# tensorlayer/TLXCV

Measured on AMD Instinct MI355X. Metric: images/sec fwd, higher is better.
Workload: dtype f16; 1 GPU; ResNet-50 fp16 forward, 224x224, batch 256 per GPU (BASELINE configs[1]); global_batch=256, per_gpu_batch=256, weights=seeded random (tlxcv_amd.seeded, seed 1), parallelism=single GPU, launch=hipGraph replay of the forward

## Files before the change

include/tlxmi.h:

```cpp
#ifndef TLXMI_H
#define TLXMI_H

#include <stddef.h>
#include <stdint.h>

#ifdef __cplusplus
extern "C" {
#endif

#define TLXMI_VERSION 101

typedef enum tlxmi_status {
    TLXMI_OK = 0,
    TLXMI_ERR_BAD_ARG = -1,
    TLXMI_ERR_UNSUPPORTED = -2,
    TLXMI_ERR_ALIGNMENT = -3,
    TLXMI_ERR_LAUNCH = -4,
    TLXMI_ERR_NO_DEVICE = -5
} tlxmi_status;

typedef enum tlxmi_dtype { TLXMI_F16 = 0, TLXMI_F32 = 1 } tlxmi_dtype;

typedef enum tlxmi_act {
    TLXMI_ACT_NONE = 0,
// ... 72 lines not shown
    int32_t N, H, W, C;
    int32_t out_h, out_w;
    int32_t kh, kw;
    int32_t out_dtype;
    int32_t layout;
    int32_t fold_b, cpad;
    int32_t normalize;
} tlxmi_preproc_desc;
size_t tlxmi_preprocess_u8_workspace_bytes(const tlxmi_preproc_desc* d);
int tlxmi_preprocess_u8(const tlxmi_preproc_desc* d, const void* images, const int32_t* xbounds, const int32_t* xk,
                        const int32_t* ybounds, const int32_t* yk, const float* mean, const float* std_, void* workspace,
                        void* out, void* stream);

int tlxmi_preprocess_linear_u8(const tlxmi_preproc_desc* d, const void* images, const int32_t* xidx, const int32_t* xcoef,
                               const int32_t* yidx, const int32_t* ycoef, const float* mean, const float* std_, void* out,
                               void* stream);

typedef struct tlxmi_seam_desc {
    int32_t dtype;
    int64_t rows;
    int32_t K1, N1, N2;
    int32_t t2_ld, skip_ld, y_ld, t1_ld;
    int32_t act;
} tlxmi_seam_desc;
int tlxmi_bottleneck_seam_supported(int dtype, int K1, int N1, int N2);
int tlxmi_bottleneck_seam_proj(const tlxmi_seam_desc* d, const void* t2, const void* w3_packed, const float* scale3,
                               const float* shift3, const void* x, const void* wd_packed, const float* scale_d,
                               const float* shift_d, void* y, const void* w1_packed, const float* scale1,
                               const float* shift1, void* t1, void* stream);
int tlxmi_bottleneck_seam(const tlxmi_seam_desc* d, const void* t2, const void* w3_packed, const float* scale3,
                          const float* shift3, const void* skip, void* y, const void* w1_packed, const float* scale1,
                          const float* shift1, void* t1, void* stream);
int tlxmi_bottleneck_seam_dec_supported(int dtype, int K1, int N1, int N2, int64_t rows, int H, int W);
int tlxmi_bottleneck_seam_dec(const tlxmi_seam_desc* d, int H, int W, const void* t2, const void* w3_packed, const float* scale3,
                              const float* shift3, const void* skip, void* y, const void* w1_packed, const float* scale1,
                              const float* shift1, void* t1, void* stream);

typedef struct tlxmi_proj_desc {
    int32_t dtype;
    int32_t N, Ho, Wo;
    int32_t K1, K2, Cout;
    int32_t H2, W2, stride;
    int32_t x_ld, x2_ld, y_ld;
    int32_t act;
    float act_param;
    uint32_t flags;
} tlxmi_proj_desc;
int tlxmi_conv1x1_proj_supported(const tlxmi_proj_desc* d, const void* x, const void* x2, const void* w_packed, const void* y);
// ... 266 lines not shown
```

tlxcv_amd/_lib.py:

```python
import ctypes as C
import os

_HERE = os.path.dirname(os.path.abspath(__file__))
LIB_PATH = os.path.join(_HERE, "libtlxmi.so")

F16, F32 = 0, 1
ACT_NONE, ACT_RELU, ACT_RELU6, ACT_LEAKY, ACT_HARDSWISH, ACT_HARDSIGMOID, ACT_GELU, ACT_SIGMOID, ACT_SILU = range(9)
EPI_RES_AFTER_ACT = 1
EPI_MAXPOOL_3S2P1 = 4
PLAN_SHARED_HALF = 0x100
PLAN_SHARED_FULL = 0x200
LAYOUT_NHWC, LAYOUT_NCHW = 0, 1


class ConvDesc(C.Structure):
    _fields_ = [(n, C.c_int32) for n in (
        "dtype", "N", "H", "W", "C", "Cout", "R", "S", "stride_h", "stride_w", "pad_h", "pad_w",
        "dil_h", "dil_w", "Ho", "Wo", "x_ld", "y_ld", "res_ld", "y_nstride", "res_nstride", "act")] + [
        ("act_param", C.c_float), ("flags", C.c_uint32)]


class DwConvDesc(C.Structure):
    _fields_ = [(n, C.c_int32) for n in (
        "dtype", "N", "H", "W", "C", "R", "S", "stride_h", "stride_w", "pad_h", "pad_w", "dil_h",
# ... 50 lines not shown
            "q_batch_stride", "q_row_stride", "k_batch_stride", "k_row_stride", "v_batch_stride", "v_row_stride",
            "out_batch_stride", "out_row_stride")]


class LevitAttnDesc(C.Structure):
    _fields_ = [(n, C.c_int32) for n in ("dtype", "B", "heads", "kd", "d", "Rq", "Rk", "stride")] + [("scale", C.c_float), ("act", C.c_int32)] + [
        (n, C.c_int64) for n in ("q_batch_stride", "q_row_stride", "q_head_stride", "k_batch_stride", "k_row_stride", "k_head_stride",
                                 "v_batch_stride", "v_row_stride", "v_head_stride", "out_batch_stride", "out_row_stride")]


class TntInnerDesc(C.Structure):
    _fields_ = [(n, C.c_int32) for n in ("dtype", "patches", "pixels", "dim", "heads", "hidden")] + [
        (n, C.c_float) for n in ("scale", "eps1", "eps2", "eps3")] + [(n, C.c_int64) for n in ("x_row_stride", "y_row_stride", "yn_row_stride")]


class GsaBlockDesc(C.Structure):
    _fields_ = [(n, C.c_int32) for n in ("dtype", "B", "Lq", "Lk", "C", "heads")] + [(n, C.c_float) for n in ("scale", "eps")] + [
        (n, C.c_int64) for n in ("x_batch_stride", "x_row_stride", "k_batch_stride", "k_row_stride", "v_batch_stride", "v_row_stride",
                                 "y_batch_stride", "y_row_stride")]


class SeamDesc(C.Structure):
    _fields_ = [("dtype", C.c_int32), ("rows", C.c_int64)] + [(n, C.c_int32) for n in (
        "K1", "N1", "N2", "t2_ld", "skip_ld", "y_ld", "t1_ld", "act")]


class ProjDesc(C.Structure):
    _fields_ = [(n, C.c_int32) for n in ("dtype", "N", "Ho", "Wo", "K1", "K2", "Cout", "H2", "W2", "stride", "x_ld", "x2_ld", "y_ld", "act")] + [
        ("act_param", C.c_float), ("flags", C.c_uint32)]


class PreprocDesc(C.Structure):
    _fields_ = [(n, C.c_int32) for n in ("N", "H", "W", "C", "out_h", "out_w", "kh", "kw", "out_dtype", "layout", "fold_b",
                                         "cpad", "normalize")]


_vp, _i, _f, _u, _l = C.c_void_p, C.c_int, C.c_float, C.c_uint32, C.c_int64

PROTOTYPES = {
    "tlxmi_nchw_to_nhwc": [_vp, _i, _vp, _i, _i, _i, _i, _i, _i, _vp],
    "tlxmi_nchw_to_nhwc_s2d": [_vp, _i, _vp, _i, _i, _i, _i, _i, _i, _i, _vp],
    "tlxmi_patchify": [_vp, _i, _vp, _i, _i, _i, _i, _i, _i, _i, _vp],
    "tlxmi_patch_embed4": [_vp, _i, _vp, _vp, _vp, _vp, _vp, _i, _i, _i, _i, _f, _vp],
    "tlxmi_patch_embed4_pos": [_vp, _i, _vp, _vp, _vp, _vp, _vp, _vp, _i, _i, _i, _i, _f, _vp],
    "tlxmi_nhwc_to_nchw": [_vp, _i, _i, _vp, _i, _i, _i, _i, _i, _vp],
    "tlxmi_pack_filter": [_vp, _vp, _i, _i, _i, _i, _i, _vp],
    "tlxmi_fold_bn": [_vp, _vp, _vp, _vp, _vp, _f, _i, _vp, _vp, _vp],
# ... 53 lines not shown
    "tlxmi_preact_conv1x1": [_i, _l, _i, _i, _i, _i, _vp, _vp, _vp, _i, _vp, _vp, _vp, _i, _vp, _vp],
    "tlxmi_lka_dw": [C.POINTER(LkaDwDesc), _vp, _vp, _vp, _vp, _vp, _vp, _vp],
    "tlxmi_lka_gate": [C.POINTER(LkaGateDesc), _vp, _vp, _vp, _vp, _vp, _vp, _vp, _vp, _vp, _vp, _vp, _vp],
    "tlxmi_mul": [_vp, _vp, _vp, _i, _l, _i, _i, _i, _i, _vp],
    "tlxmi_shuffle_unit": [C.POINTER(ShuffleUnitDesc), _vp, _vp, _vp, _vp],
    "tlxmi_shuffle_concat": [_vp, _vp, _vp, _i, _l, _i, _i, _i, _i, _vp],
    "tlxmi_ghost_module": [C.POINTER(GhostModuleDesc), _vp, _vp, _vp, _vp, _vp],
    "tlxmi_mixconv_dw": [C.POINTER(MixConvDwDesc), _vp, _vp, _vp, _vp, _vp],
}
_SPECIAL = {
    "tlxmi_version": ([], C.c_int),
    "tlxmi_last_error": ([], C.c_char_p),
    "tlxmi_device_count": ([], C.c_int),
    "tlxmi_packed_filter_bytes": ([_i, _i, _i, _i, _i], C.c_size_t),
    "tlxmi_packed_group_filter_bytes": ([_i, _i, _i, _i, _i, _i], C.c_size_t),
    "tlxmi_group_conv_chunks": ([_i, _i, _i, _i], C.c_int),
    "tlxmi_group_conv2d_small_supported": ([C.POINTER(ConvDesc), _i], C.c_int),
    "tlxmi_conv2d_maxpool_supported": ([C.POINTER(ConvDesc)], C.c_int),
    "tlxmi_conv2d_splitk_supported": ([C.POINTER(ConvDesc), _i], C.c_int),
    "tlxmi_preprocess_u8_workspace_bytes": ([C.POINTER(PreprocDesc)], C.c_size_t),
    "tlxmi_multiclass_nms_workspace_bytes": ([_i, _i], C.c_size_t),
    "tlxmi_bottleneck_seam_supported": ([_i, _i, _i, _i], C.c_int),
    "tlxmi_bottleneck_seam_dec_supported": ([_i, _i, _i, _i, _l, _i, _i], C.c_int),
    "tlxmi_conv1x1_proj_supported": ([C.POINTER(ProjDesc), _vp, _vp, _vp, _vp], C.c_int),
    "tlxmi_linear_ln_supported": ([_i, _l, _i, _i, _i, _i], C.c_int),
    "tlxmi_mlp_seam_supported": ([_i, _i, _i, _i], C.c_int),
    "tlxmi_sepconv2d_supported": ([C.POINTER(SepConvDesc)], C.c_int),
    "tlxmi_dwconv7_stats_supported": ([C.POINTER(DwConv7Desc)], C.c_int),
    "tlxmi_preact_conv1x1_supported": ([_i, _l, _i, _i, _i, _i, _i, _i], C.c_int),
    "tlxmi_sr_attention_supported": ([C.POINTER(MhaDesc)], C.c_int),
    "tlxmi_cswin_attention_supported": ([C.POINTER(CswinAttnDesc)], C.c_int),
    "tlxmi_levit_attention_supported": ([C.POINTER(LevitAttnDesc)], C.c_int),
    "tlxmi_tnt_inner_supported": ([C.POINTER(TntInnerDesc)], C.c_int),
    "tlxmi_tnt_inner_param_count": ([_i, _i], C.c_size_t),
    "tlxmi_gsa_block_supported": ([C.POINTER(GsaBlockDesc)], C.c_int),
    "tlxmi_gsa_block_param_count": ([_i], C.c_size_t),
    "tlxmi_lka_dw_supported": ([C.POINTER(LkaDwDesc)], C.c_int),
    "tlxmi_lka_gate_supported": ([C.POINTER(LkaGateDesc)], C.c_int),
    "tlxmi_shuffle_unit_supported": ([C.POINTER(ShuffleUnitDesc)], C.c_int),
    "tlxmi_shuffle_unit_param_bytes": ([_i], C.c_size_t),
    "tlxmi_ghost_module_supported": ([C.POINTER(GhostModuleDesc)], C.c_int),
    "tlxmi_ghost_module_param_bytes": ([_i, _i], C.c_size_t),
    "tlxmi_mixconv_dw_supported": ([C.POINTER(MixConvDwDesc), _i], C.c_int),
    "tlxmi_mixconv_dw_param_bytes": ([C.POINTER(MixConvDwDesc)], C.c_size_t),
}
ALL_SYMBOLS = sorted(list(PROTOTYPES) + list(_SPECIAL))
# ... 71 lines not shown
```

tlxcv_amd/csrc/block_seam.h:

```cpp
#pragma once
#include <hip/hip_runtime.h>

namespace tlxmi {

struct SeamArgs {
    const char *x, *w3, *res, *w1;
    char *y, *z;
    const float *scale3, *shift3, *scale1, *shift1;
    int M, N1;
    int x_ld, res_ld, y_ld, z_ld;
    unsigned x_bytes, w3_bytes, res_bytes, y_bytes, w1_bytes, z_bytes;
    int y_nt, z_nt;
    const char* wd;
    const float *scale_d, *shift_d;
    unsigned wd_bytes;
    int debug;
};

struct SeamDecArgs : SeamArgs {
    int HW, W;
};

bool block_seam_shape_ok(int K1, int N1, int N2);
int launch_block_seam(const SeamArgs& a, int K1, int N2, hipStream_t st);
int launch_block_seam_dec(const SeamDecArgs& a, int K1, int N2, hipStream_t st);
int launch_mlp_seam(const SeamArgs& a, int K1, int N2, hipStream_t st);

}
```

tlxcv_amd/csrc/block_seam.hip:

```cpp
#include "kernel_util.h"
#include <stdio.h>
#include "block_seam.h"
#include <type_traits>
#ifdef TLXMI_TUNING
#define TLXMI_DBG_NT(x) (x)
#else
#define TLXMI_DBG_NT(x) (false)
#endif

namespace tlxmi {

static __device__ __forceinline__ int bs_f1(int r) { return ((r >> 1) & 1) | (((r >> 4) & 3) << 1); }
static __device__ __forceinline__ int bs_f2(int r) { return (((r >> 1) & 1) << 2) | ((r >> 5) & 1); }

static __device__ __forceinline__ unsigned bs_pkrelu(unsigned v) {
    unsigned r;
    asm("v_pk_max_f16 %0, %1, 0" : "=v"(r) : "v"(v));
    return r;
}
static __device__ __forceinline__ u32x2 bs_bn_skip_relu4(f32x4 acc, f32x4 sc, f32x4 sh, half4v skip) {
    f32x2 t0 = f32x2{__builtin_fmaf(acc[0], sc[0], (float)skip[0]), __builtin_fmaf(acc[1], sc[1], (float)skip[1])};
    f32x2 t1 = f32x2{__builtin_fmaf(acc[2], sc[2], (float)skip[2]), __builtin_fmaf(acc[3], sc[3], (float)skip[3])};
    t0 += f32x2{sh[0], sh[1]};
    t1 += f32x2{sh[2], sh[3]};
// ... 263 lines not shown
        for (int h = 0; h < 2; ++h) {
            const f32x4 s0 = *reinterpret_cast<const f32x4*>(sc + 8 * h), s1 = *reinterpret_cast<const f32x4*>(sc + 8 * h + 4);
            const f32x4 h0 = *reinterpret_cast<const f32x4*>(sh + 8 * h), h1 = *reinterpret_cast<const f32x4*>(sh + 8 * h + 4);
#pragma unroll
            for (int pw = 0; pw < PW; ++pw) {
                u32x2 o0, o1;
                if constexpr (MLP) {
                    const half8v rv = __builtin_bit_cast(half8v, buf_load16(rsrd, pok[pw] ? (pix[pw] * a.res_ld + 64 * q + 16 * g + 8 * h) * 2 : BUF_OOB));
                    o0 = bs_bn_res4(acc2[4 * q + 2 * h][pw], s0, h0, half4v{rv[0], rv[1], rv[2], rv[3]});
                    o1 = bs_bn_res4(acc2[4 * q + 2 * h + 1][pw], s1, h1, half4v{rv[4], rv[5], rv[6], rv[7]});
                } else {
                    o0 = bs_bn_relu4(acc2[4 * q + 2 * h][pw], s0, h0);
                    o1 = bs_bn_relu4(acc2[4 * q + 2 * h + 1][pw], s1, h1);
                }
                const u32x4 o = u32x4{o0[0], o0[1], o1[0], o1[1]};
                if (TLXMI_DBG(a, 4)) continue;
                if (TLXMI_DBG_NT(a.z_nt)) buf_store16<BUF_NT>(zsrd, o, pok[pw] ? (pix[pw] * a.z_ld + 64 * q + 16 * g + 8 * h) * 2 : BUF_OOB);
                else buf_store16(zsrd, o, pok[pw] ? (pix[pw] * a.z_ld + 64 * q + 16 * g + 8 * h) * 2 : BUF_OOB);
            }
        }
    }
}

template <int K1, int N2, int NW>
__global__ __launch_bounds__(64 * NW, 1) void seam_pair_kernel(const SeamArgs a) {
    static_assert(N2 % 128 == 0 && NW % 2 == 0, "pairs of waves split N2 in halves of whole 64-channel blocks");
    constexpr int NT = 64 * NW;
    constexpr int IPT = 512 / NT;
    constexpr int PW = 2;
    constexpr int KS = K1 / 32;
    constexpr int CB = K1 / 64;
    constexpr int Q2 = N2 / 64;
    constexpr int NP = CB + Q2;
    constexpr int T2H = N2 / 32;
    constexpr int PANEL = 64 * 128;
    extern __shared__ __attribute__((aligned(16))) char smem[];
    char* const wbuf = smem;
    float* const tab3 = reinterpret_cast<float*>(smem + 2 * NP * PANEL);
    float* const tab1 = tab3 + 2 * a.N1;
    char* const ybuf = reinterpret_cast<char*>(tab1 + 2 * N2);

    const int t = threadIdx.x, lane = t & 63;
    const int wid = __builtin_amdgcn_readfirstlane(t >> 6);
    const int hh = wid & 1, pp = wid >> 1;
    const int fr = lane & 15, g = lane >> 4;

// ... 414 lines not shown
static int launch_seam_t(const std::conditional_t<DEC, SeamDecArgs, SeamArgs>& a, hipStream_t st) {
    constexpr int NP = K1 / 64 + N2 / 64 + (PROJ ? K1 / 64 : 0);
    const size_t lds = (size_t)2 * NP * 64 * 128 + (size_t)(2 * a.N1 + 2 * N2 + (PROJ ? 2 * a.N1 : 0)) * sizeof(float);
    if (lds > 160 * 1024) return fail(TLXMI_ERR_UNSUPPORTED, "block_seam: %zu bytes of LDS", lds);
    const void* fn = reinterpret_cast<const void*>(&seam_kernel<K1, N2, PW, NW, PROJ, WPS, MLP, DEC>);
    if (lds > 64 * 1024)
        if (int rc = raise_lds_limit(fn, 160 * 1024, "block_seam")) return rc;
    const long grid = ((long)a.M + NW * 16 * PW - 1) / (NW * 16 * PW);
    if (grid >= (1l << 31)) return fail(TLXMI_ERR_UNSUPPORTED, "block_seam: too many rows");
#ifdef TLXMI_TUNING
    if (tune_int("TLXMI_SEAM_OCC", 0)) {
        int nb = -1;
        hipError_t oe = hipOccupancyMaxActiveBlocksPerMultiprocessor(&nb, fn, 64 * NW, lds);
        fprintf(stderr, "seam<%d,%d,%d,%d,%d>: lds %zu, grid %ld, occupancy %d workgroups / CU (%s)\n", K1, N2, PW, NW, (int)PROJ, lds, grid, nb, hipGetErrorString(oe));
    }
#endif
    auto b = a;
    void* args[] = {&b};
    hipError_t e = hipLaunchKernel(fn, dim3((unsigned)grid), dim3(64 * NW), args, lds, st);
    if (e != hipSuccess) return fail(TLXMI_ERR_LAUNCH, "block_seam: HIP launch failed: %s", hipGetErrorString(e));
    return TLXMI_OK;
}

bool block_seam_shape_ok(int K1, int N1, int N2) {
    if (N1 % 64 || N1 < 64 || N1 > 2048) return false;
    if (!((K1 == 64 && (N2 == 64 || N2 == 128)) || (K1 == 128 && (N2 == 128 || N2 == 256)) || (K1 == 256 && N2 == 256))) return false;
    const size_t lds = (size_t)2 * (K1 / 64 + N2 / 64) * 64 * 128 + (size_t)(2 * N1 + 2 * N2) * sizeof(float) + (K1 == 256 ? (size_t)8 * 2 * 1024 : 0);
    return lds <= 160 * 1024;
}

int launch_mlp_seam(const SeamArgs& a0, int K1, int N2, hipStream_t st) {
    SeamArgs b = a0;
    b.z_nt = b.y_nt = 0;
    b.debug = 0;
    if (K1 == 128 && N2 == 128) return launch_seam_t<128, 128, 2, 8, false, 0, true>(b, st);
    return fail(TLXMI_ERR_UNSUPPORTED, "mlp_seam: no instantiation for %d -> N1 -> %d channels", K1, N2);
}

int launch_block_seam(const SeamArgs& a0, int K1, int N2, hipStream_t st) {
    const int vv = (int)tune_int("TLXMI_SEAM", 0);
    const int v = vv & 1;
    SeamArgs b = a0;
    b.z_nt = (vv & 2) ? 1 : 0;
    b.y_nt = (vv & 4) ? 1 : 0;
    b.debug = (int)tune_int("TLXMI_SEAM_DBG", 0);
    const SeamArgs& a = b;
    if (a.wd) {
        if (K1 == 64 && N2 == 64) return launch_seam_t<64, 64, 2, 4, true>(a, st);
        return fail(TLXMI_ERR_UNSUPPORTED, "block_seam: the projection-shortcut form is compiled for 64 -> N1 -> 64 channels");
    }
    if (vv & 16) {
        if (K1 == 64 && N2 == 64) return launch_seam_t<64, 64, 2, 4, false, 3>(a, st);
        if (K1 == 64 && N2 == 128) return launch_seam_t<64, 128, 2, 4, false, 3>(a, st);
        if (K1 == 128 && N2 == 128) return launch_seam_t<128, 128, 2, 4, false, 2>(a, st);
    }
    if (K1 == 64 && N2 == 64) return v ? launch_seam_t<64, 64, 2, 8>(a, st) : launch_seam_t<64, 64, 2, 4>(a, st);
    if (K1 == 64 && N2 == 128) return v ? launch_seam_t<64, 128, 2, 8>(a, st) : launch_seam_t<64, 128, 2, 4>(a, st);
    if (K1 == 128 && N2 == 128) return v ? launch_seam_t<128, 128, 2, 4>(a, st) : launch_seam_t<128, 128, 2, 8>(a, st);
    if (K1 == 128 && N2 == 256) return v ? launch_seam_t<128, 256, 1, 4>(a, st) : launch_seam_t<128, 256, 1, 8>(a, st);
    if (K1 == 256 && N2 == 256) {
#ifdef TLXMI_TUNING
        if (vv & 64) return launch_seam_pair_t<256, 256, 8, !SEAM_PAIR_ANTIPHASE>(a, st);
#endif
        if (!(vv & 32)) return launch_seam_pair_t<256, 256, 8, SEAM_PAIR_ANTIPHASE>(a, st);
        return v ? launch_seam_t<256, 256, 1, 4>(a, st) : launch_seam_t<256, 256, 1, 8>(a, st);
    }
    return fail(TLXMI_ERR_UNSUPPORTED, "block_seam: no instantiation for %d -> N1 -> %d channels", K1, N2);
}

static bool block_seam_dec_shape_ok(int K1, int N1, int N2) {
    return ((K1 == 64 && N1 == 256 && N2 == 128) || (K1 == 128 && N1 == 512 && N2 == 256)) && block_seam_shape_ok(K1, N1, N2);
}

int launch_block_seam_dec(const SeamDecArgs& a0, int K1, int N2, hipStream_t st) {
    SeamDecArgs b = a0;
    b.z_nt = b.y_nt = 0;
    b.debug = 0;
    if (K1 == 64 && N2 == 128) return launch_seam_t<64, 128, 2, 4, false, 0, false, true>(b, st);
    if (K1 == 128 && N2 == 256) return launch_seam_t<128, 256, 1, 8, false, 0, false, true>(b, st);
    return fail(TLXMI_ERR_UNSUPPORTED, "block_seam_dec: no instantiation for %d -> N1 -> %d channels", K1, N2);
}

}

using namespace tlxmi;

extern "C" int tlxmi_bottleneck_seam_supported(int dtype, int K1, int N1, int N2) {
    return dtype == TLXMI_F16 && block_seam_shape_ok(K1, N1, N2) ? 1 : 0;
}

static int seam_impl(const tlxmi_seam_desc* d, const void* t2, const void* w3_packed, const float* scale3,
                     const float* shift3, const void* skip, void* y, const void* w1_packed, const float* scale1,
                     const float* shift1, void* t1, void* stream, const void* wd_packed, const float* scale_d, const float* shift_d) {
    TLXMI_REQUIRE(d && t2 && w3_packed && skip && y && w1_packed && t1, TLXMI_ERR_BAD_ARG, "bottleneck_seam: null argument");
    TLXMI_REQUIRE(d->dtype == TLXMI_F16, TLXMI_ERR_UNSUPPORTED, "bottleneck_seam: fp16 only (the fp32 parity mode runs the two convolutions)");
    TLXMI_REQUIRE(d->rows > 0 && d->K1 > 0 && d->N1 > 0 && d->N2 > 0, TLXMI_ERR_BAD_ARG, "bottleneck_seam: bad extent");
    if (!block_seam_shape_ok(d->K1, d->N1, d->N2))
        return fail(TLXMI_ERR_UNSUPPORTED, "bottleneck_seam: no kernel for %d -> %d -> %d channels", d->K1, d->N1, d->N2);
    TLXMI_REQUIRE(d->t2_ld >= d->K1 && d->skip_ld >= (wd_packed ? d->K1 : d->N1) && d->y_ld >= d->N1 && d->t1_ld >= d->N2, TLXMI_ERR_BAD_ARG, "bottleneck_seam: row stride below the channel count");
    TLXMI_REQUIRE(!wd_packed || (aligned16(wd_packed) && d->K1 == 64 && d->N2 == 64), TLXMI_ERR_UNSUPPORTED, "bottleneck_seam_proj: 64 -> N1 -> 64 channels only");
    TLXMI_REQUIRE(d->t2_ld % 8 == 0 && d->skip_ld % 8 == 0 && d->y_ld % 8 == 0 && d->t1_ld % 8 == 0 && aligned16(t2) && aligned16(skip) && aligned16(y) &&
                      aligned16(t1) && aligned16(w3_packed) && aligned16(w1_packed),
                  TLXMI_ERR_ALIGNMENT, "bottleneck_seam: rows must be whole 16-byte chunks");
    TLXMI_REQUIRE(d->act == TLXMI_ACT_RELU, TLXMI_ERR_UNSUPPORTED, "bottleneck_seam: ReLU after both convolutions only");
    const long long rows = d->rows;
    const long long big = (1ll << 31);
    TLXMI_REQUIRE(rows * d->t2_ld * 2 < big && rows * d->skip_ld * 2 < big && rows * d->y_ld * 2 < big && rows * d->t1_ld * 2 < big && rows < big,
                  TLXMI_ERR_UNSUPPORTED, "bottleneck_seam: a tensor exceeds the 2 GiB the 32-bit buffer offsets address");
    SeamArgs a;
    a.x = (const char*)t2; a.w3 = (const char*)w3_packed; a.res = (const char*)skip; a.w1 = (const char*)w1_packed;
    a.y = (char*)y; a.z = (char*)t1;
    a.scale3 = scale3; a.shift3 = shift3; a.scale1 = scale1; a.shift1 = shift1;
    a.M = (int)rows; a.N1 = d->N1;
    a.x_ld = d->t2_ld; a.res_ld = d->skip_ld; a.y_ld = d->y_ld; a.z_ld = d->t1_ld;
    a.x_bytes = (unsigned)(rows * d->t2_ld * 2); a.res_bytes = (unsigned)(rows * d->skip_ld * 2);
    a.y_bytes = (unsigned)(rows * d->y_ld * 2); a.z_bytes = (unsigned)(rows * d->t1_ld * 2);
    a.wd = (const char*)wd_packed; a.scale_d = scale_d; a.shift_d = shift_d;
    a.wd_bytes = wd_packed ? (unsigned)(((size_t)(d->N1 + 127) / 128 * 128) * (size_t)d->K1 * 2) : 0u;
    a.w3_bytes = (unsigned)(((size_t)(d->N1 + 127) / 128 * 128) * (size_t)d->K1 * 2);
    a.w1_bytes = (unsigned)(((size_t)(d->N2 + 127) / 128 * 128) * (size_t)d->N1 * 2);
    const int rc = launch_block_seam(a, d->K1, d->N2, as_stream(stream));
    if (rc != TLXMI_OK) return rc;
    return check_launch("bottleneck_seam");
}

extern "C" int tlxmi_bottleneck_seam(const tlxmi_seam_desc* d, const void* t2, const void* w3_packed, const float* scale3,
                                     const float* shift3, const void* skip, void* y, const void* w1_packed, const float* scale1,
                                     const float* shift1, void* t1, void* stream) {
    return seam_impl(d, t2, w3_packed, scale3, shift3, skip, y, w1_packed, scale1, shift1, t1, stream, nullptr, nullptr, nullptr);
}

extern "C" int tlxmi_bottleneck_seam_proj(const tlxmi_seam_desc* d, const void* t2, const void* w3_packed, const float* scale3,
                                          const float* shift3, const void* x, const void* wd_packed, const float* scale_d,
                                          const float* shift_d, void* y, const void* w1_packed, const float* scale1,
                                          const float* shift1, void* t1, void* stream) {
    TLXMI_REQUIRE(wd_packed, TLXMI_ERR_BAD_ARG, "bottleneck_seam_proj: null shortcut filter");
    return seam_impl(d, t2, w3_packed, scale3, shift3, x, y, w1_packed, scale1, shift1, t1, stream, wd_packed, scale_d, shift_d);
}

static long long seam_dec_rows(long long rows, int H, int W) { return rows / ((long long)H * W) * ((H + 1) / 2) * ((W + 1) / 2); }

extern "C" int tlxmi_bottleneck_seam_dec_supported(int dtype, int K1, int N1, int N2, int64_t rows, int H, int W) {
    if (dtype != TLXMI_F16 || !block_seam_dec_shape_ok(K1, N1, N2) || rows <= 0 || H <= 0 || W <= 0) return 0;
    const long long big = (1ll << 31), hw = (long long)H * W;
// ... 12 lines not shown
    const long long big = (1ll << 31), rows = d->rows, hw = (long long)H * W;
    TLXMI_REQUIRE(hw < big && rows % hw == 0, TLXMI_ERR_BAD_ARG, "bottleneck_seam_dec: rows is not a whole number of H x W images");
    TLXMI_REQUIRE(d->t2_ld >= d->K1 && d->skip_ld >= d->N1 && d->y_ld >= d->N1 && d->t1_ld >= d->N2, TLXMI_ERR_BAD_ARG, "bottleneck_seam_dec: row stride below the channel count");
    TLXMI_REQUIRE(d->t2_ld % 8 == 0 && d->skip_ld % 8 == 0 && d->y_ld % 8 == 0 && d->t1_ld % 8 == 0 && aligned16(t2) && aligned16(skip) && aligned16(y) &&
                      aligned16(t1) && aligned16(w3_packed) && aligned16(w1_packed),
                  TLXMI_ERR_ALIGNMENT, "bottleneck_seam_dec: rows must be whole 16-byte chunks");
    TLXMI_REQUIRE(d->act == TLXMI_ACT_RELU, TLXMI_ERR_UNSUPPORTED, "bottleneck_seam_dec: ReLU after both convolutions only");
    const long long yrows = seam_dec_rows(rows, H, W);
    TLXMI_REQUIRE(rows * d->t2_ld * 2 < big && rows * d->skip_ld * 2 < big && yrows * d->y_ld * 2 < big && rows * d->t1_ld * 2 < big,
                  TLXMI_ERR_UNSUPPORTED, "bottleneck_seam_dec: a tensor exceeds the 2 GiB the 32-bit buffer offsets address");
    SeamDecArgs a;
    a.x = (const char*)t2; a.w3 = (const char*)w3_packed; a.res = (const char*)skip; a.w1 = (const char*)w1_packed;
    a.y = (char*)y; a.z = (char*)t1;
    a.scale3 = scale3; a.shift3 = shift3; a.scale1 = scale1; a.shift1 = shift1;
    a.M = (int)rows; a.N1 = d->N1;
    a.x_ld = d->t2_ld; a.res_ld = d->skip_ld; a.y_ld = d->y_ld; a.z_ld = d->t1_ld;
    a.x_bytes = (unsigned)(rows * d->t2_ld * 2); a.res_bytes = (unsigned)(rows * d->skip_ld * 2);
    a.y_bytes = (unsigned)(yrows * d->y_ld * 2); a.z_bytes = (unsigned)(rows * d->t1_ld * 2);
    a.wd = nullptr; a.scale_d = a.shift_d = nullptr; a.wd_bytes = 0;
    a.w3_bytes = (unsigned)(((size_t)(d->N1 + 127) / 128 * 128) * (size_t)d->K1 * 2);
    a.w1_bytes = (unsigned)(((size_t)(d->N2 + 127) / 128 * 128) * (size_t)d->N1 * 2);
    a.y_nt = a.z_nt = 0; a.debug = 0;
    a.HW = (int)hw; a.W = W;
    const int rc = launch_block_seam_dec(a, d->K1, d->N2, as_stream(stream));
    if (rc != TLXMI_OK) return rc;
    return check_launch("bottleneck_seam_dec");
}

extern "C" int tlxmi_mlp_seam_supported(int dtype, int K, int hidden, int N) {
    return (dtype == TLXMI_F16 && K == 128 && N == 128 && hidden % 64 == 0 && hidden >= 64 && hidden <= 2048 && block_seam_shape_ok(K, hidden, N)) ? 1 : 0;
}

extern "C" int tlxmi_mlp_seam(int dtype, int64_t rows, int K, int hidden, int N, const void* x, int x_ld, const void* w1_packed, const float* bias1,
                              const void* w2_packed, const float* bias2, const void* res, int res_ld, void* out, int out_ld, void* stream) {
    TLXMI_REQUIRE(x && w1_packed && w2_packed && res && out, TLXMI_ERR_BAD_ARG, "mlp_seam: null argument");
    if (!tlxmi_mlp_seam_supported(dtype, K, hidden, N)) return fail(TLXMI_ERR_UNSUPPORTED, "mlp_seam: no kernel for %d -> %d -> %d", K, hidden, N);
    TLXMI_REQUIRE(rows > 0 && x_ld >= K && res_ld >= N && out_ld >= N, TLXMI_ERR_BAD_ARG, "mlp_seam: bad extent");
    TLXMI_REQUIRE(x_ld % 8 == 0 && res_ld % 8 == 0 && out_ld % 8 == 0 && aligned16(x) && aligned16(res) && aligned16(out) && aligned16(w1_packed) && aligned16(w2_packed),
                  TLXMI_ERR_ALIGNMENT, "mlp_seam: rows must be whole 16-byte chunks");
    const long long big = (1ll << 31);
    TLXMI_REQUIRE(rows * x_ld * 2 < big && rows * res_ld * 2 < big && rows * out_ld * 2 < big, TLXMI_ERR_UNSUPPORTED, "mlp_seam: a tensor exceeds 2 GiB");
    SeamArgs a;
    a.x = (const char*)x; a.w3 = (const char*)w1_packed; a.res = (const char*)res; a.w1 = (const char*)w2_packed;
    a.y = nullptr; a.z = (char*)out;
    a.scale3 = nullptr; a.shift3 = bias1; a.scale1 = nullptr; a.shift1 = bias2;
    a.M = (int)rows; a.N1 = hidden;
    a.x_ld = x_ld; a.res_ld = res_ld; a.y_ld = 0; a.z_ld = out_ld;
// ... 10 lines not shown
```

tlxcv_amd/engine.py:

```python
import ctypes as C
import threading

import torch

from . import _lib
from ._lib import (ACT_GELU, ACT_HARDSIGMOID, ACT_HARDSWISH, ACT_LEAKY, ACT_NONE, ACT_RELU, ACT_RELU6,
                   ACT_SIGMOID, ACT_SILU, EPI_RES_AFTER_ACT, F16, F32)

EPI_RES_BCAST_N = 2

_precision = torch.float16

_options = {"splitk": True,
            "attn_comb": True,
            "seams": True,
            "seam256": True,
            "proj_fold": 7,
            "seam_decimate": True,
            "two_streams": True,
            "conv_splitk": True,
            "patch_linear": True,
            "patch_embed4": True,
            "mlp_seam": True,
            "lnfold": True,
# ... 554 lines not shown


def bottleneck_seam_supported(K1, N1, N2, dtype):
    return bool(_lib.load().tlxmi_bottleneck_seam_supported(dt_code(dtype), int(K1), int(N1), int(N2)))


def bottleneck_seam_dec_supported(K1, N1, N2, rows, H, W, dtype):
    return bool(_lib.load().tlxmi_bottleneck_seam_dec_supported(dt_code(dtype), int(K1), int(N1), int(N2), int(rows), int(H), int(W)))


def bottleneck_seam(t2, pk3, scale3, shift3, skip, pk1, scale1, shift1, proj=None, y_stride2=False):
    need_gpu(t2, "input")
    N, H, W, ld = t2.shape
    if y_stride2 and proj is not None:
        raise RuntimeError("bottleneck_seam: no decimated form of the projection-shortcut seam")
    if skip.shape[:3] != t2.shape[:3] or skip.dtype != t2.dtype or not skip.is_contiguous() or not t2.is_contiguous():
        raise RuntimeError("bottleneck_seam: t2 / skip must be dense NHWC maps of one dtype and extent")
    y = torch.empty((N, (H + 1) // 2, (W + 1) // 2, pk3.Cout) if y_stride2 else (N, H, W, pk3.Cout), dtype=t2.dtype, device=t2.device)
    t1 = torch.empty((N, H, W, pk1.Cout), dtype=t2.dtype, device=t2.device)
    rows = N * H * W
    if getattr(_tls, "act_max", None) is not None:
        _note_act(t2.numel() * t2.element_size(), skip.numel() * skip.element_size(), y.numel() * y.element_size(), t1.numel() * t1.element_size())
    d = _lib.SeamDesc(dtype=dt_code(t2.dtype), rows=rows, K1=pk3.Cin, N1=pk3.Cout, N2=pk1.Cout, t2_ld=ld, skip_ld=skip.shape[-1],
                      y_ld=pk3.Cout, t1_ld=pk1.Cout, act=ACT_RELU)
    if y_stride2:
        name = "tlxmi_bottleneck_seam_dec"
        args = (C.byref(d), H, W, _p(t2), _p(pk3.buf), _p(scale3), _p(shift3), _p(skip), _p(y), _p(pk1.buf), _p(scale1), _p(shift1), _p(t1), _stream())
    elif proj is None:
        name = "tlxmi_bottleneck_seam"
        args = (C.byref(d), _p(t2), _p(pk3.buf), _p(scale3), _p(shift3), _p(skip), _p(y), _p(pk1.buf), _p(scale1), _p(shift1), _p(t1), _stream())
    else:
        name = "tlxmi_bottleneck_seam_proj"
        pkd, sd, hd = proj
        args = (C.byref(d), _p(t2), _p(pk3.buf), _p(scale3), _p(shift3), _p(skip), _p(pkd.buf), _p(sd), _p(hd), _p(y), _p(pk1.buf), _p(scale1),
                _p(shift1), _p(t1), _stream())
    if _probe is None:
        _lib.call(name, *args)
        return y, t1
    es = t2.element_size()
    skip_ch = pk3.Cout if proj is None else proj[0].Cin
    alg_bytes = (rows * (pk3.Cin + skip_ch + pk1.Cout) + y.numel() + pk3.Cout * pk3.Cin + pk1.Cout * pk1.Cin) * es
    flops = 2 * rows * (pk3.Cout * pk3.Cin + pk1.Cout * pk1.Cin + (0 if proj is None else pk3.Cout * proj[0].Cin))
    e0, e1 = torch.cuda.Event(enable_timing=True), torch.cuda.Event(enable_timing=True)
    e0.record()
    _lib.call(name, *args)
    e1.record()
    _probe.append((e0, e1, alg_bytes, flops, (N, H, W, pk3.Cin, pk3.Cout, pk1.Cout, "seam+dec" if y_stride2 else "seam" if proj is None else "seam+proj", True)))
# ... 1745 lines not shown
```

Measured before the change: 80760 images/sec.

## Add persistent LDS-resident-weight bottleneck seam kernel for K1=64 stages

Adds a persistent kernel for the bottleneck seam (1x1 conv3 + BN + skip + ReLU fused with the next block's 1x1 conv1). It stages all filter panels and BN tables into up to 160 KiB of LDS once per workgroup, then grid-strides over 32-row tiles with prefetched activations and skip data. The aim is to stop reloading weights per tile and to cut launch/occupancy overhead for the K1=64 plain, projection and decimated forms. It is selected by default unless a shared-plan flag is set. The cost is one resident workgroup per CU and a large LDS footprint, which may limit latency hiding.

```diff
diff --git a/include/tlxmi.h b/include/tlxmi.h
--- a/include/tlxmi.h
+++ b/include/tlxmi.h
@@ -118,8 +118,10 @@
     int32_t K1, N1, N2;
     int32_t t2_ld, skip_ld, y_ld, t1_ld;
     int32_t act;
+    uint32_t flags;
 } tlxmi_seam_desc;
 int tlxmi_bottleneck_seam_supported(int dtype, int K1, int N1, int N2);
+int tlxmi_bottleneck_seam_resident(int dtype, int K1, int N1, int N2, int form);
 int tlxmi_bottleneck_seam_proj(const tlxmi_seam_desc* d, const void* t2, const void* w3_packed, const float* scale3,
                                const float* shift3, const void* x, const void* wd_packed, const float* scale_d,
                                const float* shift_d, void* y, const void* w1_packed, const float* scale1,
diff --git a/tlxcv_amd/_lib.py b/tlxcv_amd/_lib.py
--- a/tlxcv_amd/_lib.py
+++ b/tlxcv_amd/_lib.py
@@ -96,7 +96,7 @@
 
 class SeamDesc(C.Structure):
     _fields_ = [("dtype", C.c_int32), ("rows", C.c_int64)] + [(n, C.c_int32) for n in (
-        "K1", "N1", "N2", "t2_ld", "skip_ld", "y_ld", "t1_ld", "act")]
+        "K1", "N1", "N2", "t2_ld", "skip_ld", "y_ld", "t1_ld", "act")] + [("flags", C.c_uint32)]
 
 
 class ProjDesc(C.Structure):
@@ -196,6 +196,7 @@
     "tlxmi_multiclass_nms_workspace_bytes": ([_i, _i], C.c_size_t),
     "tlxmi_bottleneck_seam_supported": ([_i, _i, _i, _i], C.c_int),
     "tlxmi_bottleneck_seam_dec_supported": ([_i, _i, _i, _i, _l, _i, _i], C.c_int),
+    "tlxmi_bottleneck_seam_resident": ([_i, _i, _i, _i, _i], C.c_int),
     "tlxmi_conv1x1_proj_supported": ([C.POINTER(ProjDesc), _vp, _vp, _vp, _vp], C.c_int),
     "tlxmi_linear_ln_supported": ([_i, _l, _i, _i, _i, _i], C.c_int),
     "tlxmi_mlp_seam_supported": ([_i, _i, _i, _i], C.c_int),
diff --git a/tlxcv_amd/csrc/block_seam.h b/tlxcv_amd/csrc/block_seam.h
--- a/tlxcv_amd/csrc/block_seam.h
+++ b/tlxcv_amd/csrc/block_seam.h
@@ -22,8 +22,8 @@
 };
 
 bool block_seam_shape_ok(int K1, int N1, int N2);
-int launch_block_seam(const SeamArgs& a, int K1, int N2, hipStream_t st);
-int launch_block_seam_dec(const SeamDecArgs& a, int K1, int N2, hipStream_t st);
+int launch_block_seam(const SeamArgs& a, int K1, int N2, bool shared, hipStream_t st);
+int launch_block_seam_dec(const SeamDecArgs& a, int K1, int N2, bool shared, hipStream_t st);
 int launch_mlp_seam(const SeamArgs& a, int K1, int N2, hipStream_t st);
 
 }
diff --git a/tlxcv_amd/csrc/block_seam.hip b/tlxcv_amd/csrc/block_seam.hip
--- a/tlxcv_amd/csrc/block_seam.hip
+++ b/tlxcv_amd/csrc/block_seam.hip
@@ -309,6 +309,264 @@
     }
 }
 
+template <int N2, int NW, bool PROJ, bool DEC>
+__global__ __launch_bounds__(64 * NW, 1) void seam_res_kernel(const std::conditional_t<DEC, SeamDecArgs, SeamArgs> a) {
+    static_assert(!(PROJ && DEC), "one form at a time");
+    static_assert(NW >= 8, "the first 512 threads stage the filters");
+    constexpr int K1 = 64;
+    constexpr int PW = 2;
+    constexpr int NT = 64 * NW;
+    constexpr int KS = K1 / 32;
+    constexpr int Q2 = N2 / 64;
+    constexpr int NP = 1 + Q2 + (PROJ ? 1 : 0);
+    constexpr int T2 = N2 / 16;
+    constexpr int PANEL = 64 * 128;
+    extern __shared__ __attribute__((aligned(16))) char smem[];
+    const int nch = a.N1 >> 6;
+    char* const wbuf = smem;
+    float* const tab3 = reinterpret_cast<float*>(smem + nch * NP * PANEL);
+    float* const tab1 = tab3 + 2 * a.N1;
+    float* const tabd = tab1 + 2 * N2;
+
+    const int t = threadIdx.x, lane = t & 63;
+    const int wid = __builtin_amdgcn_readfirstlane(t >> 6);
+    const int fr = lane & 15, g = lane >> 4;
+
+    const __amdgpu_buffer_rsrc_t xsrd = buf_srd(a.x, a.x_bytes), w3srd = buf_srd(a.w3, a.w3_bytes), w1srd = buf_srd(a.w1, a.w1_bytes);
+    const __amdgpu_buffer_rsrc_t rsrd = buf_srd(a.res, a.res_bytes), ysrd = buf_srd(a.y, a.y_bytes), zsrd = buf_srd(a.z, a.z_bytes);
+    const __amdgpu_buffer_rsrc_t wdsrd = buf_srd(PROJ ? a.wd : a.w3, PROJ ? a.wd_bytes : 0u);
+
+    const int ntile = (a.M + 16 * PW - 1) / (16 * PW);
+    const int nwv = (int)gridDim.x * NW;
+    int tile = TLXMI_DBG(a, 64) ? (int)blockIdx.x * NW + wid : wid * (int)gridDim.x + (int)blockIdx.x;
+
+    auto load_x = [&](int tl, u32x4 (&xv)[KS][PW], u32x4 (&xpv)[PROJ ? KS : 1][PW]) {
+#pragma unroll
+        for (int pw = 0; pw < PW; ++pw) {
+            const int p = tl * (16 * PW) + 16 * pw + fr;
+            const bool ok = p < a.M;
+#pragma unroll
+            for (int ks = 0; ks < KS; ++ks) {
+                xv[ks][pw] = buf_load16(xsrd, ok ? (p * a.x_ld + 32 * ks + 8 * g) * 2 : BUF_OOB);
+                if constexpr (PROJ) xpv[ks][pw] = buf_load16(rsrd, ok ? (p * a.res_ld + 32 * ks + 8 * g) * 2 : BUF_OOB);
+            }
+        }
+    };
+    int ptile = tile, pc = 0;
+    int roff[PW];
+    auto skip_rows = [&]() {
+#pragma unroll
+        for (int pw = 0; pw < PW; ++pw) {
+            const int p = ptile * (16 * PW) + 16 * pw + fr;
+            roff[pw] = (p < a.M && !TLXMI_DBG(a, 2)) ? (p * a.res_ld + 16 * g) * 2 : BUF_OOB;
+        }
+    };
+    auto skip_load = [&](u32x4 (&s)[PW][2]) {
+        if constexpr (PROJ) return;
+#pragma unroll
+        for (int pw = 0; pw < PW; ++pw)
+#pragma unroll
+            for (int h = 0; h < 2; ++h) s[pw][h] = buf_load16(rsrd, roff[pw] + (64 * pc + 8 * h) * 2);
+        if (++pc == nch) {
+            pc = 0;
+            ptile += nwv;
+            skip_rows();
+        }
+    };
+
+    u32x4 xf[KS][PW], xpf[PROJ ? KS : 1][PW];
+    load_x(tile, xf, xpf);
+    u32x4 sk[PW][2], sk1[PW][2];
+    if constexpr (!PROJ) skip_rows();
+    skip_load(sk);
+    skip_load(sk1);
+
+    if (t < 512) {
+        const int srow = t >> 3, sslot = t & 7;
+        const int sl1 = sslot ^ bs_f1(srow), sl2 = sslot ^ bs_f2(srow);
+#pragma unroll 1
+        for (int c0 = 0; c0 < nch; c0 += 4) {
+            u32x4 st[4][NP];
+#pragma unroll
+            for (int e = 0; e < 4; ++e) {
+                const int c = c0 + e, dead = c < nch ? 0 : BUF_OOB;
+                st[e][0] = buf_load16(w3srd, (((64 * c + srow) * K1 + 8 * sl1) * 2) | dead);
+#pragma unroll
+                for (int q = 0; q < Q2; ++q) st[e][1 + q] = buf_load16(w1srd, (((64 * q + srow) * a.N1 + 64 * c + 8 * sl2) * 2) | dead);
+                if constexpr (PROJ) st[e][1 + Q2] = buf_load16(wdsrd, (((64 * c + srow) * K1 + 8 * sl1) * 2) | dead);
+            }
+#pragma unroll
+            for (int e = 0; e < 4; ++e) {
+                if (c0 + e < nch) {
+#pragma unroll
+                    for (int j = 0; j < NP; ++j) *reinterpret_cast<u32x4*>(wbuf + ((c0 + e) * NP + j) * PANEL + t * 16) = st[e][j];
+                }
+            }
+        }
+    }
+    for (int i = t; i < a.N1; i += NT) {
+        tab3[i] = a.scale3 ? a.scale3[i] : 1.f;
+        tab3[a.N1 + i] = a.shift3 ? a.shift3[i] : 0.f;
+    }
+    for (int i = t; i < N2; i += NT) {
+        tab1[i] = a.scale1 ? a.scale1[i] : 1.f;
+        tab1[N2 + i] = a.shift1 ? a.shift1[i] : 0.f;
+    }
+    if constexpr (PROJ) {
+        for (int i = t; i < a.N1; i += NT) {
+            tabd[i] = a.scale_d ? a.scale_d[i] : 1.f;
+            tabd[a.N1 + i] = a.shift_d ? a.shift_d[i] : 0.f;
+        }
+    }
+    __syncthreads();
+
+    const int arow = 16 * (fr >> 2) + (fr & 3);
+    int a1off[4], a2off[4];
+#pragma unroll
+    for (int ci = 0; ci < 4; ++ci) {
+        const int r = arow + 4 * ci;
+        a1off[ci] = r * 128 + ((g ^ bs_f1(r)) << 4);
+        a2off[ci] = r * 128 + (((2 * g) ^ bs_f2(r)) << 4);
+    }
+
+#pragma unroll 1
+    for (; tile < ntile; tile += nwv) {
+        int yoff[PW], zoff[PW];
+#pragma unroll
+        for (int pw = 0; pw < PW; ++pw) {
+            const int p = tile * (16 * PW) + 16 * pw + fr;
+            const bool ok = p < a.M;
+            zoff[pw] = ok ? (p * a.z_ld + 16 * g) * 2 : BUF_OOB;
+            if constexpr (DEC) {
+                const int Wc = (a.W + 1) >> 1, HcWc = ((a.HW / a.W + 1) >> 1) * Wc;
+                const int n = p / a.HW, r = p - n * a.HW, h = r / a.W, w = r - h * a.W;
+                yoff[pw] = (ok && !((h | w) & 1)) ? ((n * HcWc + (h >> 1) * Wc + (w >> 1)) * a.y_ld + 16 * g) * 2 : BUF_OOB;
+            } else {
+                yoff[pw] = ok ? (p * a.y_ld + 16 * g) * 2 : BUF_OOB;
+            }
+        }
+        u32x4 xfn[KS][PW], xpfn[PROJ ? KS : 1][PW];
+        load_x(tile + nwv, xfn, xpfn);
+
+        f32x4 acc2[T2][PW];
+#pragma unroll
+        for (int tt = 0; tt < T2; ++tt)
+#pragma unroll
+            for (int pw = 0; pw < PW; ++pw) acc2[tt][pw] = f32x4{0.f, 0.f, 0.f, 0.f};
+
+#pragma unroll 1
+        for (int c = 0; c < nch; ++c) {
+            const char* const wb = wbuf + c * NP * PANEL;
+            u32x4 sk2[PW][2];
+            skip_load(sk2);
+
+            f32x4 acc1[4][PW];
+#pragma unroll
+            for (int ci = 0; ci < 4; ++ci) {
+#pragma unroll
+                for (int pw = 0; pw < PW; ++pw) acc1[ci][pw] = f32x4{0.f, 0.f, 0.f, 0.f};
+                if (TLXMI_DBG(a, 16)) continue;
+#pragma unroll
+                for (int ks = 0; ks < KS; ++ks) {
+                    const u32x4 af = *reinterpret_cast<const u32x4*>(wb + (a1off[ci] ^ ((ks & 1) << 6)));
+#pragma unroll
+                    for (int pw = 0; pw < PW; ++pw) acc1[ci][pw] = Mma<half_t>::run(af, xf[ks][pw], acc1[ci][pw]);
+                }
+            }
+            f32x4 accd[PROJ ? 4 : 1][PW];
+            if constexpr (PROJ) {
+#pragma unroll
+                for (int ci = 0; ci < 4; ++ci) {
+#pragma unroll
+                    for (int pw = 0; pw < PW; ++pw) accd[ci][pw] = f32x4{0.f, 0.f, 0.f, 0.f};
+#pragma unroll
+                    for (int ks = 0; ks < KS; ++ks) {
+                        const u32x4 af = *reinterpret_cast<const u32x4*>(wb + (1 + Q2) * PANEL + (a1off[ci] ^ ((ks & 1) << 6)));
+#pragma unroll
+                        for (int pw = 0; pw < PW; ++pw) accd[ci][pw] = Mma<half_t>::run(af, xpf[ks][pw], accd[ci][pw]);
+                    }
+                }
+            }
+
+            u32x4 yf[PW][2];
+            {
+                const float* sc = tab3 + 64 * c + 16 * g;
+                const float* sh = sc + a.N1;
+#pragma unroll
+                for (int h = 0; h < 2; ++h) {
+                    const f32x4 s0 = *reinterpret_cast<const f32x4*>(sc + 8 * h), s1 = *reinterpret_cast<const f32x4*>(sc + 8 * h + 4);
+                    const f32x4 h0 = *reinterpret_cast<const f32x4*>(sh + 8 * h), h1 = *reinterpret_cast<const f32x4*>(sh + 8 * h + 4);
+                    f32x4 d0 = s0, d1 = s0, e0 = s0, e1 = s0;
+                    if constexpr (PROJ) {
+                        const float* scd = tabd + 64 * c + 16 * g + 8 * h;
+                        d0 = *reinterpret_cast<const f32x4*>(scd); d1 = *reinterpret_cast<const f32x4*>(scd + 4);
+                        e0 = *reinterpret_cast<const f32x4*>(scd + a.N1); e1 = *reinterpret_cast<const f32x4*>(scd + a.N1 + 4);
+                    }
+#pragma unroll
+                    for (int pw = 0; pw < PW; ++pw) {
+                        half8v rv;
+                        if constexpr (PROJ) {
+#pragma unroll
+                            for (int e = 0; e < 4; ++e) {
+                                rv[e] = (half_t)(accd[2 * h][pw][e] * d0[e] + e0[e]);
+                                rv[4 + e] = (half_t)(accd[2 * h + 1][pw][e] * d1[e] + e1[e]);
+                            }
+                        } else {
+                            rv = __builtin_bit_cast(half8v, sk[pw][h]);
+                        }
+                        const u32x2 o0 = bs_bn_skip_relu4(acc1[2 * h][pw], s0, h0, half4v{rv[0], rv[1], rv[2], rv[3]});
+                        const u32x2 o1 = bs_bn_skip_relu4(acc1[2 * h + 1][pw], s1, h1, half4v{rv[4], rv[5], rv[6], rv[7]});
+                        yf[pw][h] = u32x4{o0[0], o0[1], o1[0], o1[1]};
+                        if (TLXMI_DBG(a, 1)) continue;
+                        buf_store16(ysrd, yf[pw][h], yoff[pw] + (64 * c + 8 * h) * 2);
+                    }
+                }
+            }
+
+#pragma unroll
+            for (int tt = 0; tt < T2; ++tt) {
+                if (TLXMI_DBG(a, 16)) continue;
+#pragma unroll
+                for (int s = 0; s < 2; ++s) {
+                    const u32x4 af = *reinterpret_cast<const u32x4*>(wb + (1 + (tt >> 2)) * PANEL + (a2off[tt & 3] ^ (s << 4)));
+#pragma unroll
+                    for (int pw = 0; pw < PW; ++pw) acc2[tt][pw] = Mma<half_t>::run(af, yf[pw][s], acc2[tt][pw]);
+                }
+            }
+            if constexpr (!PROJ) {
+#pragma unroll
+                for (int pw = 0; pw < PW; ++pw)
+#pragma unroll
+                    for (int h = 0; h < 2; ++h) { sk[pw][h] = sk1[pw][h]; sk1[pw][h] = sk2[pw][h]; }
+            }
+        }
+
+#pragma unroll
+        for (int q = 0; q < Q2; ++q) {
+            const float* sc = tab1 + 64 * q + 16 * g;
+            const float* sh = sc + N2;
+#pragma unroll
+            for (int h = 0; h < 2; ++h) {
+                const f32x4 s0 = *reinterpret_cast<const f32x4*>(sc + 8 * h), s1 = *reinterpret_cast<const f32x4*>(sc + 8 * h + 4);
+                const f32x4 h0 = *reinterpret_cast<const f32x4*>(sh + 8 * h), h1 = *reinterpret_cast<const f32x4*>(sh + 8 * h + 4);
+#pragma unroll
+                for (int pw = 0; pw < PW; ++pw) {
+                    const u32x2 o0 = bs_bn_relu4(acc2[4 * q + 2 * h][pw], s0, h0), o1 = bs_bn_relu4(acc2[4 * q + 2 * h + 1][pw], s1, h1);
+                    if (TLXMI_DBG(a, 4)) continue;
+                    buf_store16(zsrd, u32x4{o0[0], o0[1], o1[0], o1[1]}, zoff[pw] + (64 * q + 8 * h) * 2);
+                }
+            }
+        }
+#pragma unroll
+        for (int ks = 0; ks < KS; ++ks)
+#pragma unroll
+            for (int pw = 0; pw < PW; ++pw) {
+                xf[ks][pw] = xfn[ks][pw];
+                if constexpr (PROJ) xpf[ks][pw] = xpfn[ks][pw];
+            }
+    }
+}
+
 template <int K1, int N2, int NW>
 __global__ __launch_bounds__(64 * NW, 1) void seam_pair_kernel(const SeamArgs a) {
     static_assert(N2 % 128 == 0 && NW % 2 == 0, "pairs of waves split N2 in halves of whole 64-channel blocks");
@@ -769,6 +1027,37 @@
     return TLXMI_OK;
 }
 
+static size_t seam_res_lds(int K1, int N1, int N2, bool proj) {
+    return ((size_t)K1 * N1 * (proj ? 2 : 1) + (size_t)N1 * N2) * 2 + (size_t)(2 * N1 + 2 * N2 + (proj ? 2 * N1 : 0)) * sizeof(float);
+}
+enum { SEAM_PLAIN = 0, SEAM_PROJ = 1, SEAM_DEC = 2 };
+static bool seam_res_ok(int K1, int N1, int N2, int form) {
+    if (K1 != 64 || N1 < 64 || N1 % 64 || N2 != (form == SEAM_DEC ? 128 : 64)) return false;
+    return seam_res_lds(K1, N1, N2, form == SEAM_PROJ) <= 160 * 1024;
+}
+
+template <int N2, int NW, bool PROJ, bool DEC> static int launch_seam_res_t(const std::conditional_t<DEC, SeamDecArgs, SeamArgs>& a, hipStream_t st) {
+    const size_t lds = seam_res_lds(64, a.N1, N2, PROJ);
+    if (lds > 160 * 1024) return fail(TLXMI_ERR_UNSUPPORTED, "block_seam: %zu bytes of LDS", lds);
+    const void* fn = reinterpret_cast<const void*>(&seam_res_kernel<N2, NW, PROJ, DEC>);
+    if (lds > 64 * 1024)
+        if (int rc = raise_lds_limit(fn, 160 * 1024, "block_seam")) return rc;
+    const long tiles = ((long)a.M + 31) / 32, want = (tiles + NW - 1) / NW;
+    long grid = device_cus();
+    const long forced = tune_int("TLXMI_SEAM_GRID", 0);
+    if (forced > 0) grid = forced;
+    if (grid > want) grid = want;
+    auto b = a;
+    void* args[] = {&b};
+    hipError_t e = hipLaunchKernel(fn, dim3((unsigned)grid), dim3(64 * NW), args, lds, st);
+    if (e != hipSuccess) return fail(TLXMI_ERR_LAUNCH, "block_seam: HIP launch failed: %s", hipGetErrorString(e));
+    return TLXMI_OK;
+}
+template <int N2, bool PROJ, bool DEC> static int launch_seam_res(const std::conditional_t<DEC, SeamDecArgs, SeamArgs>& a, int vv, hipStream_t st) {
+    (void)vv;
+    return launch_seam_res_t<N2, 8, PROJ, DEC>(a, st);
+}
+
 bool block_seam_shape_ok(int K1, int N1, int N2) {
     if (N1 % 64 || N1 < 64 || N1 > 2048) return false;
     if (!((K1 == 64 && (N2 == 64 || N2 == 128)) || (K1 == 128 && (N2 == 128 || N2 == 256)) || (K1 == 256 && N2 == 256))) return false;
@@ -784,7 +1073,7 @@
     return fail(TLXMI_ERR_UNSUPPORTED, "mlp_seam: no instantiation for %d -> N1 -> %d channels", K1, N2);
 }
 
-int launch_block_seam(const SeamArgs& a0, int K1, int N2, hipStream_t st) {
+int launch_block_seam(const SeamArgs& a0, int K1, int N2, bool shared, hipStream_t st) {
     const int vv = (int)tune_int("TLXMI_SEAM", 0);
     const int v = vv & 1;
     SeamArgs b = a0;
@@ -792,7 +1081,9 @@
     b.y_nt = (vv & 4) ? 1 : 0;
     b.debug = (int)tune_int("TLXMI_SEAM_DBG", 0);
     const SeamArgs& a = b;
+    const bool res = !(vv & 128) && (!shared || (vv & 2048));
     if (a.wd) {
+        if (res && !(vv & 512) && seam_res_ok(K1, a.N1, N2, SEAM_PROJ)) return launch_seam_res<64, true, false>(a, vv, st);
         if (K1 == 64 && N2 == 64) return launch_seam_t<64, 64, 2, 4, true>(a, st);
         return fail(TLXMI_ERR_UNSUPPORTED, "block_seam: the projection-shortcut form is compiled for 64 -> N1 -> 64 channels");
     }
@@ -801,6 +1092,7 @@
         if (K1 == 64 && N2 == 128) return launch_seam_t<64, 128, 2, 4, false, 3>(a, st);
         if (K1 == 128 && N2 == 128) return launch_seam_t<128, 128, 2, 4, false, 2>(a, st);
     }
+    if (res && !(vv & 256) && seam_res_ok(K1, a.N1, N2, SEAM_PLAIN)) return launch_seam_res<64, false, false>(a, vv, st);
     if (K1 == 64 && N2 == 64) return v ? launch_seam_t<64, 64, 2, 8>(a, st) : launch_seam_t<64, 64, 2, 4>(a, st);
     if (K1 == 64 && N2 == 128) return v ? launch_seam_t<64, 128, 2, 8>(a, st) : launch_seam_t<64, 128, 2, 4>(a, st);
     if (K1 == 128 && N2 == 128) return v ? launch_seam_t<128, 128, 2, 4>(a, st) : launch_seam_t<128, 128, 2, 8>(a, st);
@@ -819,10 +1111,12 @@
     return ((K1 == 64 && N1 == 256 && N2 == 128) || (K1 == 128 && N1 == 512 && N2 == 256)) && block_seam_shape_ok(K1, N1, N2);
 }
 
-int launch_block_seam_dec(const SeamDecArgs& a0, int K1, int N2, hipStream_t st) {
+int launch_block_seam_dec(const SeamDecArgs& a0, int K1, int N2, bool shared, hipStream_t st) {
     SeamDecArgs b = a0;
     b.z_nt = b.y_nt = 0;
-    b.debug = 0;
+    b.debug = (int)tune_int("TLXMI_SEAM_DBG", 0);
+    const int vv = (int)tune_int("TLXMI_SEAM", 0);
+    if (!(vv & (128 | 1024)) && (!shared || (vv & 2048)) && seam_res_ok(K1, b.N1, N2, SEAM_DEC)) return launch_seam_res<128, false, true>(b, vv, st);
     if (K1 == 64 && N2 == 128) return launch_seam_t<64, 128, 2, 4, false, 0, false, true>(b, st);
     if (K1 == 128 && N2 == 256) return launch_seam_t<128, 256, 1, 8, false, 0, false, true>(b, st);
     return fail(TLXMI_ERR_UNSUPPORTED, "block_seam_dec: no instantiation for %d -> N1 -> %d channels", K1, N2);
@@ -831,6 +1125,12 @@
 }
 
 using namespace tlxmi;
+
+extern "C" int tlxmi_bottleneck_seam_resident(int dtype, int K1, int N1, int N2, int form) {
+    if (dtype != TLXMI_F16 || form < SEAM_PLAIN || form > SEAM_DEC) return 0;
+    if (form == SEAM_DEC ? !block_seam_dec_shape_ok(K1, N1, N2) : !block_seam_shape_ok(K1, N1, N2)) return 0;
+    return seam_res_ok(K1, N1, N2, form) ? 1 : 0;
+}
 
 extern "C" int tlxmi_bottleneck_seam_supported(int dtype, int K1, int N1, int N2) {
     return dtype == TLXMI_F16 && block_seam_shape_ok(K1, N1, N2) ? 1 : 0;
@@ -866,7 +1166,7 @@
     a.wd_bytes = wd_packed ? (unsigned)(((size_t)(d->N1 + 127) / 128 * 128) * (size_t)d->K1 * 2) : 0u;
     a.w3_bytes = (unsigned)(((size_t)(d->N1 + 127) / 128 * 128) * (size_t)d->K1 * 2);
     a.w1_bytes = (unsigned)(((size_t)(d->N2 + 127) / 128 * 128) * (size_t)d->N1 * 2);
-    const int rc = launch_block_seam(a, d->K1, d->N2, as_stream(stream));
+    const int rc = launch_block_seam(a, d->K1, d->N2, (d->flags & (TLXMI_PLAN_SHARED_HALF | TLXMI_PLAN_SHARED_FULL)) != 0, as_stream(stream));
     if (rc != TLXMI_OK) return rc;
     return check_launch("bottleneck_seam");
 }
@@ -925,7 +1225,7 @@
     a.w1_bytes = (unsigned)(((size_t)(d->N2 + 127) / 128 * 128) * (size_t)d->N1 * 2);
     a.y_nt = a.z_nt = 0; a.debug = 0;
     a.HW = (int)hw; a.W = W;
-    const int rc = launch_block_seam_dec(a, d->K1, d->N2, as_stream(stream));
+    const int rc = launch_block_seam_dec(a, d->K1, d->N2, (d->flags & (TLXMI_PLAN_SHARED_HALF | TLXMI_PLAN_SHARED_FULL)) != 0, as_stream(stream));
     if (rc != TLXMI_OK) return rc;
     return check_launch("bottleneck_seam_dec");
 }
diff --git a/tlxcv_amd/engine.py b/tlxcv_amd/engine.py
--- a/tlxcv_amd/engine.py
+++ b/tlxcv_amd/engine.py
@@ -600,7 +600,7 @@
     if getattr(_tls, "act_max", None) is not None:
         _note_act(t2.numel() * t2.element_size(), skip.numel() * skip.element_size(), y.numel() * y.element_size(), t1.numel() * t1.element_size())
     d = _lib.SeamDesc(dtype=dt_code(t2.dtype), rows=rows, K1=pk3.Cin, N1=pk3.Cout, N2=pk1.Cout, t2_ld=ld, skip_ld=skip.shape[-1],
-                      y_ld=pk3.Cout, t1_ld=pk1.Cout, act=ACT_RELU)
+                      y_ld=pk3.Cout, t1_ld=pk1.Cout, act=ACT_RELU, flags=plan_flags())
     if y_stride2:
         name = "tlxmi_bottleneck_seam_dec"
         args = (C.byref(d), H, W, _p(t2), _p(pk3.buf), _p(scale3), _p(shift3), _p(skip), _p(y), _p(pk1.buf), _p(scale1), _p(shift1), _p(t1), _stream())
```

Result: no change. 80650 images/sec (-0.1%).
